# hkust-vgd/nerfstyle

Hardware: AMD Instinct MI355X
Metric: train Mrays/sec (higher is better)
Workload: dtype f16

## Files before the change

nerfstyle_amd/csrc/field_bwd_gout.hip:

```cpp
#include "field_bwd.h"

template <int CD>
__device__ __forceinline__ void field_wgrad_mfma4(f4v &c0, f4v &c1, f4v &c2, f4v &c3, s4v a0, s4v b0, s4v a1, s4v b1, s4v a2,
                                                  s4v b2, s4v a3, s4v b3) {
    if (CD == NSR_F16)
        asm volatile("s_nop 1\n\t"
                     "v_mfma_f32_16x16x16_f16 %0, %4, %5, %0\n\t"
                     "v_mfma_f32_16x16x16_f16 %1, %6, %7, %1\n\t"
                     "v_mfma_f32_16x16x16_f16 %2, %8, %9, %2\n\t"
                     "v_mfma_f32_16x16x16_f16 %3, %10, %11, %3"
                     : "+a"(c0), "+a"(c1), "+a"(c2), "+a"(c3)
                     : "v"(a0), "v"(b0), "v"(a1), "v"(b1), "v"(a2), "v"(b2), "v"(a3), "v"(b3));
    else
        asm volatile("s_nop 1\n\t"
                     "v_mfma_f32_16x16x16_bf16 %0, %4, %5, %0\n\t"
                     "v_mfma_f32_16x16x16_bf16 %1, %6, %7, %1\n\t"
                     "v_mfma_f32_16x16x16_bf16 %2, %8, %9, %2\n\t"
                     "v_mfma_f32_16x16x16_bf16 %3, %10, %11, %3"
                     : "+a"(c0), "+a"(c1), "+a"(c2), "+a"(c3)
                     : "v"(a0), "v"(b0), "v"(a1), "v"(b1), "v"(a2), "v"(b2), "v"(a3), "v"(b3));
}
template <int NT>
__device__ __forceinline__ void field_wgrad_settle(f4v (&acc)[NT]) {
    static_assert(NT % 4 == 0, "accumulators come in blocks of four");
#pragma unroll
    for (int k = 0; k < NT; k += 4)
        asm volatile("s_nop 15\n\ts_nop 3" : "+a"(acc[k]), "+a"(acc[k + 1]), "+a"(acc[k + 2]), "+a"(acc[k + 3]));
}
template <int CD, int NG, int NA>
__device__ __forceinline__ void field_wgrad(f4v (&acc)[NG * NA], const s4v (&Gt)[NG], const s4v (&At)[NA]) {
    static_assert((NG * NA) % 4 == 0, "accumulators come in blocks of four");
#pragma unroll
    for (int j = 0; j < NG * NA; j += 4)
        field_wgrad_mfma4<CD>(acc[j], acc[j + 1], acc[j + 2], acc[j + 3], Gt[j / NA], At[j % NA], Gt[(j + 1) / NA],
                              At[(j + 1) % NA], Gt[(j + 2) / NA], At[(j + 2) % NA], Gt[(j + 3) / NA], At[(j + 3) % NA]);
}

constexpr int TR_DEPTH = 4;
template <int CD>
__device__ __forceinline__ void field_tr4p(const s8v (&x)[2], s4v ident, s4v (&out)[4]) {
    const s4v in[4] = {mm_lo(x[0]), mm_hi(x[0]), mm_lo(x[1]), mm_hi(x[1])};
    mm_transpose16_n<CD, 4, TR_DEPTH>(in, ident, out);
}
template <int CD>
__device__ __forceinline__ void field_tr5p(const s8v (&x)[2], s4v y, s4v ident, s4v (&out)[4], s4v (&yt)[1]) {
    const s4v in[5] = {mm_lo(x[0]), mm_hi(x[0]), mm_lo(x[1]), mm_hi(x[1]), y};
    s4v o[5];
    mm_transpose16_n<CD, 5, TR_DEPTH>(in, ident, o);
    out[0] = o[0]; out[1] = o[1]; out[2] = o[2]; out[3] = o[3]; yt[0] = o[4];
}
template <int CD>
__device__ __forceinline__ void field_tr6p(const s8v (&x)[2], s4v y, s4v z, s4v ident, s4v (&out)[4], s4v (&yt)[1], s4v (&zt)[1]) {
    const s4v in[6] = {mm_lo(x[0]), mm_hi(x[0]), mm_lo(x[1]), mm_hi(x[1]), y, z};
    s4v o[6];
    mm_transpose16_n<CD, 6, TR_DEPTH>(in, ident, o);
    out[0] = o[0]; out[1] = o[1]; out[2] = o[2]; out[3] = o[3]; yt[0] = o[4]; zt[0] = o[5];
}

template <typename TT, int CD, bool FEATS, bool DIRS = false>
__global__ void __launch_bounds__(BWD_THREADS)
k_field_bwd_gout(FieldBwdArgsOf<DIRS> b) {
    constexpr int FWT = FW_IMAGE<DIRS>;
    const float *const dirs = field_dirs_of(b);
    extern __shared__ __attribute__((aligned(16))) char smem[];
    short *wl = reinterpret_cast<short *>(smem);
    short *wt = wl + FWT;
    NsrLevel *lds_lv = reinterpret_cast<NsrLevel *>(smem + (size_t)(FWT + BW_TOTAL) * 2);
    const FieldArgs &a = b.f;
    field_build_fw<CD, false, DIRS>(wl, a.params);
    field_build_bw<CD>(wt, a.params);
    if (threadIdx.x < 16) lds_lv[threadIdx.x] = a.lv[threadIdx.x];
    __syncthreads();

    const uint32_t Mc = FIELD_COUNT(a);
    const uint32_t ntiles = (Mc + 15) / 16;
    const int lane = threadIdx.x & 63, wave = __builtin_amdgcn_readfirstlane((int)(threadIdx.x >> 6));
    const int s = lane & 15, g = lane >> 4;
    const TT *tables = reinterpret_cast<const TT *>(a.tables);
    const uint32_t lb = field_logical_block();
    const uint32_t tpb = (ntiles + gridDim.x - 1) / gridDim.x;
    const uint32_t t_begin = lb * tpb;
    const uint32_t t_end = min(t_begin + tpb, ntiles);
    const s4v ident = mm_identity_frag<CD>(lane);
    const int nc = (int)b.nc;
    const bool td = b.train_density != 0, tc = b.train_color != 0;
    f4v w_r3[4], w_r2[16], w_r1[4], w_c1b[4], w_c1a[8], w_k2[4], w_k1[8], w_d2[4], w_d1[8];
    f4v w_sh[4];
    {
        const f4v z = {0.f, 0.f, 0.f, 0.f};
        if constexpr (DIRS) { w_sh[0] = z; w_sh[1] = z; w_sh[2] = z; w_sh[3] = z; }
#pragma unroll
        for (int q4 = 0; q4 < 4; q4++) { w_r3[q4] = z; w_r1[q4] = z; w_c1b[q4] = z; w_k2[q4] = z; w_d2[q4] = z; }
#pragma unroll
        for (int q8 = 0; q8 < 8; q8++) { w_c1a[q8] = z; w_k1[q8] = z; w_d1[q8] = z; }
#pragma unroll
        for (int q16 = 0; q16 < 16; q16++) w_r2[q16] = z;
    }

    struct TileIn {
        float x0, x1, x2;
        s8v xd, xc;
        float gsig;
        float grgb[4];
    };
    auto fetch_idx = [&](uint32_t tile) -> uint32_t {
        const uint32_t m = tile * 16 + s;
        if (a.perm) return a.perm[min(m, Mc - 1u)];
        return m < Mc ? m : 0u;
    };
    auto load_tile = [&](uint32_t tile, uint32_t buf_idx) {
        TileIn r;
        const size_t mc = buf_idx;
        r.x0 = a.xyzs[mc * 3 + 0];
        r.x1 = a.xyzs[mc * 3 + 1];
        r.x2 = a.xyzs[mc * 3 + 2];
        r.gsig = b.grad_sigmas[mc];
        const float *gp = b.grad_rgbs + mc * a.C_ch;
        if (a.C_ch == 8) {
            const float4 t4 = reinterpret_cast<const float4 *>(gp)[g & 1];
            r.grgb[0] = t4.x; r.grgb[1] = t4.y; r.grgb[2] = t4.z; r.grgb[3] = t4.w;
        } else {
#pragma unroll
            for (int e = 0; e < 4; e++) r.grgb[e] = gp[(uint32_t)(4 * g + e) < a.C_ch ? 4 * g + e : 0];
        }
        if (FEATS) {
            const s8v *fi = reinterpret_cast<const s8v *>(a.feats) + ((size_t)tile * 64 + lane) * 2;
            r.xd = fi[0];
            r.xc = fi[1];
        }
        return r;
    };
    const uint32_t wchunk = (t_end > t_begin ? (t_end - t_begin + BWD_THREADS / 64 - 1) / (BWD_THREADS / 64) : 0u);
    const uint32_t w_begin = min(t_begin + wave * wchunk, t_end), w_end = min(w_begin + wchunk, t_end);
    TileIn cur;
    uint32_t idx_cur = 0, idx_next = 0;
    if (w_begin < w_end) {
        idx_cur = fetch_idx(w_begin);
        cur = load_tile(w_begin, idx_cur);
        idx_next = w_begin + 1 < w_end ? fetch_idx(w_begin + 1) : idx_cur;
    }
    float4 gout_v[4];
    uint32_t gout_m = 0;
    bool gout_valid = false;
    auto gout_store = [&]() {
        if (gout_valid) {
#pragma unroll
            for (int i = 0; i < 4; i++) {
                const int lv_i = (i < 2 ? 2 * g : 8 + 2 * g) + (i & 1);
                b.gout[(size_t)gout_m * 16 + lv_i] = gout_v[i];
            }
        }
        gout_valid = false;
    };
    bool ch_on[4], ch_rgb[4], ch_cls[4];
#pragma unroll
    for (int e = 0; e < 4; e++) {
        const int ch = 4 * g + e;
        ch_on[e] = a.C_ch == 8 ? g < 2 : (uint32_t)ch < a.C_ch;
        ch_rgb[e] = (uint32_t)ch < a.C_ch && ch < 3;
        ch_cls[e] = (uint32_t)ch < a.C_ch && ch >= 3;
    }
    s8v wq[4];
    s4v wq16[4];
    mm_queue32<4>(wq, wl + FW_D1, lane);
    for (uint32_t tile = w_begin; tile < w_end; tile++) {
        const uint32_t m = tile * 16 + s;
        const bool valid = m < Mc;
        asm volatile("" ::: "memory");
        asm volatile("" :: "v"(cur.x0), "v"(cur.x1), "v"(cur.x2), "v"(cur.gsig), "v"(cur.grgb[0]), "v"(cur.grgb[1]),
                     "v"(cur.grgb[2]), "v"(cur.grgb[3]), "v"(cur.xd), "v"(cur.xc), "v"(idx_next));
        float dv[3] = {0.f, 0.f, 0.f};
        if constexpr (DIRS) { dv[0] = dirs[(size_t)idx_cur * 3 + 0]; dv[1] = dirs[(size_t)idx_cur * 3 + 1]; dv[2] = dirs[(size_t)idx_cur * 3 + 2]; }
        const float u0 = field_unit(cur.x0, a.bmin[0], a.bsize[0]);
        const float u1 = field_unit(cur.x1, a.bmin[1], a.bsize[1]);
        const float u2 = field_unit(cur.x2, a.bmin[2], a.bsize[2]);
        const bool live = valid && (u0 >= 0 && u0 <= 1 && u1 >= 0 && u1 <= 1 && u2 >= 0 && u2 <= 1);
        const float cur_gsig = valid ? cur.gsig : 0.f;
        float cur_grgb[4];
#pragma unroll
        for (int e = 0; e < 4; e++) cur_grgb[e] = (valid && ch_on[e]) ? cur.grgb[e] : 0.f;
        if (!FEATS) field_encode<TT, CD, false>(lds_lv, tables, u0, u1, u2, live, g, cur.xd, cur.xc, a.fast_levels);

        f4v gxd[2], gxc[2];
        s8v xd[1] = {cur.xd}, xc[1] = {cur.xc};
        f4v h[4];
        s8v hd[2], hk[2], hc[2], hr1[2], hr2[2];
        f4v logit[1], c1[1], rgb[1];
        mm_layer32_q<CD, 4, 1>(wq, wl + FW_D1, lane, xd, h);
        mm_queue32<2>(wq, wl + FW_D2, lane);
        gout_store();
        const TileIn nxt = load_tile(min(tile + 1, w_end - 1), idx_next);
        const uint32_t idx_nn = fetch_idx(min(tile + 2, w_end - 1));
        mm_pack64<CD, true, true>(h, hd);
        mm_layer32_q<CD, 1, 2>(wq, wl + FW_D2, lane, hd, logit);
        mm_queue32<4>(wq, wl + FW_K1, lane);
        mm_layer32_q<CD, 4, 1>(wq, wl + FW_K1, lane, xc, h);
        mm_queue32<4>(wq, wl + FW_C1A, lane);
        mm_pack64<CD, true, true>(h, hk);
        mm_layer32_q<CD, 4, 1>(wq, wl + FW_C1A, lane, xc, h);
        mm_queue32<2>(wq, wl + FW_C1B, lane);
        mm_pack64<CD, true, true>(h, hc);
        mm_layer32_q<CD, 1, 2>(wq, wl + FW_C1B, lane, hc, c1);
        s4v shb = {};
        if constexpr (DIRS) mm_queue32<4>(wq, wl + FW_R1, lane);
        else mm_queue16<4>(wq16, wl + FW_R1, lane);
        const s4v c1b = mm_round4<CD, false>(c1[0]);
        if constexpr (DIRS) {
            shb = mm_round4<CD, false>(field_sh4(g, dv[0], dv[1], dv[2]));
            const s8v b1[1] = {mm_cat(c1b, shb)};
            mm_layer32_q<CD, 4, 1>(wq, wl + FW_R1, lane, b1, h);
        } else {
            mm_layer16_q<CD, 4>(wq16, c1b, h);
        }
        mm_queue32<8>(wq, wl + FW_R2, lane);
        mm_pack64<CD, true, true>(h, hr1);
        mm_layer32_q<CD, 4, 2>(wq, wl + FW_R2, lane, hr1, h);
        mm_queue32<2>(wq, wl + FW_R3, lane);
        mm_pack64<CD, true, true>(h, hr2);
        mm_layer32_q<CD, 1, 2>(wq, wl + FW_R3, lane, hr2, rgb);
        mm_queue16<4>(wq16, wt + BW_R3T, lane);

        s4v dyd, dyr, dyk;
        {
            float gd[4] = {0.f, 0.f, 0.f, 0.f}, gr[4] = {0.f, 0.f, 0.f, 0.f}, gk[4] = {0.f, 0.f, 0.f, 0.f};
            {
                const float x = logit[0][0];
                const float d = cur_gsig * a.density_scale * expf(fminf(fmaxf(x, -15.0f), 15.0f));
                gd[0] = (valid && g == 0) ? d : 0.f;
            }
#pragma unroll
            for (int e = 0; e < 4; e++) {
                const float gv = cur_grgb[e];
                if (e < 3) {
                    const float sg = field_sigmoid(rgb[0][e]);
                    const float d = gv * sg * (1.0f - sg);
                    gr[e] = (valid && ch_rgb[e]) ? d : 0.f;
                }
                gk[e] = (valid && ch_cls[e]) ? gv : 0.f;
            }
#pragma unroll
            for (int e = 0; e < 4; e++) { dyd[e] = MM<CD>::cvt(gd[e]); dyr[e] = MM<CD>::cvt(gr[e]); dyk[e] = MM<CD>::cvt(gk[e]); }
        }

        s8v g2[2], g1[2];
        s4v gc1;
        {
            mm_layer16_q<CD, 4>(wq16, dyr, h);
            mm_queue32<8>(wq, wt + BW_R2T, lane);
            field_mask_pack<CD, true>(h, hr2, g2);
            mm_layer32_q<CD, 4, 2>(wq, wt + BW_R2T, lane, g2, h);
            mm_queue32<2>(wq, wt + BW_R1T, lane);
            field_mask_pack<CD, true>(h, hr1, g1);
            f4v t1[1];
            mm_layer32_q<CD, 1, 2>(wq, wt + BW_R1T, lane, g1, t1);
            mm_queue16<4>(wq16, wt + BW_C1BT, lane);
            gc1 = mm_round4<CD, false>(t1[0]);
            s4v hr2t[4], hr1t[4], g2t[4], g1t[4], dyrt[1], c1t[1];
            field_tr5p<CD>(hr2, dyr, ident, hr2t, dyrt);
            field_wgrad<CD>(w_r3, dyrt, hr2t);
            field_tr4p<CD>(g2, ident, g2t);
            field_tr4p<CD>(hr1, ident, hr1t);
            field_wgrad<CD>(w_r2, g2t, hr1t);
            if constexpr (DIRS) {
                s4v sht[1];
                field_tr6p<CD>(g1, c1b, shb, ident, g1t, c1t, sht);
                field_wgrad<CD>(w_r1, g1t, c1t);
                field_wgrad<CD>(w_sh, g1t, sht);
            } else {
                field_tr5p<CD>(g1, c1b, ident, g1t, c1t);
                field_wgrad<CD>(w_r1, g1t, c1t);
            }
        }
        s4v xct[2], xdt[2];
        {
            const s8v xcd[2] = {xc[0], xd[0]};
            s4v xt[4];
            field_tr4p<CD>(xcd, ident, xt);
            xct[0] = xt[0]; xct[1] = xt[1]; xdt[0] = xt[2]; xdt[1] = xt[3];
        }

        {
            s8v gh[2];
            s4v ght[4], hct[4], gc1t[1];
            mm_layer16_q<CD, 4>(wq16, gc1, h);
            mm_queue32<4>(wq, wt + BW_C1AT, lane);
            field_mask_pack<CD, true>(h, hc, gh);
            mm_layer32_q<CD, 2, 2>(wq, wt + BW_C1AT, lane, gh, gxc);
            mm_queue16<4>(wq16, wt + BW_K2T, lane);
            field_tr5p<CD>(hc, gc1, ident, hct, gc1t);
            field_wgrad<CD>(w_c1b, gc1t, hct);
            field_tr4p<CD>(gh, ident, ght);
            field_wgrad<CD>(w_c1a, ght, xct);
        }
        {
            s8v gh[2];
            s4v ght[4], hkt[4], dykt[1];
            mm_layer16_q<CD, 4>(wq16, dyk, h);
            mm_queue32<4>(wq, wt + BW_K1T, lane);
            field_mask_pack<CD, true>(h, hk, gh);
            mm_layer32_q<CD, 2, 2, true>(wq, wt + BW_K1T, lane, gh, gxc);
            mm_queue16<4>(wq16, wt + BW_D2T, lane);
            field_tr5p<CD>(hk, dyk, ident, hkt, dykt);
            field_wgrad<CD>(w_k2, dykt, hkt);
            field_tr4p<CD>(gh, ident, ght);
            field_wgrad<CD>(w_k1, ght, xct);
        }
        {
            s8v gh[2];
            s4v ght[4], hdt[4], dydt[1];
            mm_layer16_q<CD, 4>(wq16, dyd, h);
            mm_queue32<4>(wq, wt + BW_D1T, lane);
            field_mask_pack<CD, true>(h, hd, gh);
            mm_layer32_q<CD, 2, 2>(wq, wt + BW_D1T, lane, gh, gxd);
            mm_queue32<4>(wq, wl + FW_D1, lane);
            field_tr5p<CD>(hd, dyd, ident, hdt, dydt);
            field_wgrad<CD>(w_d2, dydt, hdt);
            field_tr4p<CD>(gh, ident, ght);
            field_wgrad<CD>(w_d1, ght, xdt);
        }

        if (td || tc) {
            float4 sg[4];
#pragma unroll
            for (int i = 0; i < 4; i++) {
                const int t = i >> 1, e0 = 2 * (i & 1);
                sg[i] = live ? make_float4(gxd[t][e0], gxd[t][e0 + 1], gxc[t][e0], gxc[t][e0 + 1]) : make_float4(0.f, 0.f, 0.f, 0.f);
            }
#pragma unroll
            for (int i = 0; i < 4; i++) gout_v[i] = sg[i];
            gout_m = idx_cur;
            gout_valid = valid;
        }
        cur = nxt;
        idx_cur = idx_next; idx_next = idx_nn;
    }
    gout_store();
        field_wgrad_settle(w_r3); field_wgrad_settle(w_r2); field_wgrad_settle(w_r1); field_wgrad_settle(w_c1b);
        field_wgrad_settle(w_c1a); field_wgrad_settle(w_k2); field_wgrad_settle(w_k1); field_wgrad_settle(w_d2);
        field_wgrad_settle(w_d1);
        if constexpr (DIRS) field_wgrad_settle(w_sh);

    if (b.grad_mlp) {
        f4v *const red = reinterpret_cast<f4v *>(smem);
#define NSR_RED_ALL(OP)                                                                                              \
        OP(w_r3, 0, 4) OP(w_r2, 4, 16) OP(w_r1, 20, 4) OP(w_c1b, 24, 4) OP(w_c1a, 28, 8) OP(w_k2, 36, 4) OP(w_k1, 40, 8)     \
        OP(w_d2, 48, 4) OP(w_d1, 52, 8)
        __syncthreads();
        for (int w = 0; w < BWD_THREADS / 64; w++) {
            if (wave == w) {
                if (w == 0) {
#define NSR_RED_ST(arr, base, n) _Pragma("unroll") for (int i = 0; i < n; i++) red[((base) + i) * 64 + lane] = arr[i];
                    NSR_RED_ALL(NSR_RED_ST)
                    if constexpr (DIRS) { NSR_RED_ST(w_sh, 60, 4) }
#undef NSR_RED_ST
                } else {
#define NSR_RED_ADD(arr, base, n) _Pragma("unroll") for (int i = 0; i < n; i++) red[((base) + i) * 64 + lane] += arr[i];
                    NSR_RED_ALL(NSR_RED_ADD)
                    if constexpr (DIRS) { NSR_RED_ADD(w_sh, 60, 4) }
#undef NSR_RED_ADD
                }
            }
            __syncthreads();
        }
        if (wave == 0) {
#define NSR_RED_LD(arr, base, n) _Pragma("unroll") for (int i = 0; i < n; i++) arr[i] = red[((base) + i) * 64 + lane];
            NSR_RED_ALL(NSR_RED_LD)
            if constexpr (DIRS) { NSR_RED_LD(w_sh, 60, 4) }
#undef NSR_RED_LD
            float *gm = b.grad_mlp;
            if constexpr (DIRS) field_wgrad_flush<4, 1>(gm + P_SH, 16, 0, 64, w_sh, lane);
            field_wgrad_flush<1, 4>(gm + P_R3, 64, 0, 3, w_r3, lane);
            field_wgrad_flush<4, 4>(gm + P_R2, 64, 0, 64, w_r2, lane);
            field_wgrad_flush<4, 1>(gm + P_R1, 16, 0, 64, w_r1, lane);
            field_wgrad_flush<1, 4>(gm + P_C1B, 64, 0, 16, w_c1b, lane);
            field_wgrad_flush<4, 2>(gm + P_C1A, 32, 0, 64, w_c1a, lane);
            field_wgrad_flush<1, 4>(gm + P_K2, 64, CLASS_ROW_SHIFT, nc, w_k2, lane);
            field_wgrad_flush<4, 2>(gm + P_K1, 32, 0, 64, w_k1, lane);
            field_wgrad_flush<1, 4>(gm + P_D2, 64, 0, 1, w_d2, lane);
            field_wgrad_flush<4, 2>(gm + P_D1, 32, 0, 64, w_d1, lane);
        }
#undef NSR_RED_ALL
    }
}

constexpr int COLOR_THREADS = 512;
template <int CD, bool DIRS = false>
__global__ void __launch_bounds__(COLOR_THREADS)
k_field_bwd_color(FieldBwdArgsOf<DIRS> b) {
    constexpr int AHEAD = 4;
    const float *const dirs = field_dirs_of(b);
    extern __shared__ __attribute__((aligned(16))) char smem[];
    short *wl = reinterpret_cast<short *>(smem);
    short *wt = wl + FW_IMAGE<DIRS>;
    const FieldArgs &a = b.f;
    field_build_fw<CD, false, DIRS>(wl, a.params);
    field_build_bw<CD>(wt, a.params);
    __syncthreads();
    const uint32_t Mc = FIELD_COUNT(a);
    const uint32_t ntiles = (Mc + 15) / 16;
    const int lane = threadIdx.x & 63, wave = threadIdx.x >> 6;
    const int s = lane & 15, g = lane >> 4;
    const uint32_t lb = field_logical_block();
    const uint32_t tpb = (ntiles + gridDim.x - 1) / gridDim.x;
    const uint32_t t_begin = lb * tpb;
    const uint32_t t_end = min(t_begin + tpb, ntiles);
    for (uint32_t tile = t_begin + wave; tile < t_end; tile += COLOR_THREADS / 64) {
        const uint32_t mpos = tile * 16 + s;
        const bool valid = mpos < Mc;
        const uint32_t m = a.perm[min(mpos, Mc - 1u)];
        const float u0 = field_unit(a.xyzs[(size_t)m * 3 + 0], a.bmin[0], a.bsize[0]);
        const float u1 = field_unit(a.xyzs[(size_t)m * 3 + 1], a.bmin[1], a.bsize[1]);
        const float u2 = field_unit(a.xyzs[(size_t)m * 3 + 2], a.bmin[2], a.bsize[2]);
        const bool live = valid && field_in_unit_cube(u0, u1, u2);
        float grgb[4];
        {
            const float *gp = b.grad_rgbs + (size_t)m * a.C_ch;
            if (a.C_ch == 8) {
                const float4 t4 = reinterpret_cast<const float4 *>(gp)[g & 1];
                grgb[0] = t4.x; grgb[1] = t4.y; grgb[2] = t4.z; grgb[3] = t4.w;
            } else {
#pragma unroll
                for (int e = 0; e < 4; e++) grgb[e] = gp[(uint32_t)(4 * g + e) < a.C_ch ? 4 * g + e : 0];
            }
#pragma unroll
            for (int e = 0; e < 4; e++)
                if (!(valid && (a.C_ch == 8 ? g < 2 : (uint32_t)(4 * g + e) < a.C_ch))) grgb[e] = 0.f;
        }
        const s8v xc[1] = {(reinterpret_cast<const s8v *>(a.feats) + ((size_t)tile * 64 + lane) * 2)[1]};
        f4v h[4];
        s8v hk[2], hc[2], hr1[2], hr2[2];
        f4v c1[1], rgb[1];
        mm_layer32<CD, 4, 1, AHEAD>(wl + FW_K1, lane, xc, h);
        mm_pack64<CD, true, true>(h, hk);
        mm_layer32<CD, 4, 1, AHEAD>(wl + FW_C1A, lane, xc, h);
        mm_pack64<CD, true, true>(h, hc);
        mm_layer32<CD, 1, 2, AHEAD>(wl + FW_C1B, lane, hc, c1);
        const s4v c1b = mm_round4<CD, false>(c1[0]);
        if constexpr (DIRS) {
            const s8v b1[1] = {mm_cat(c1b, field_sh_frag<CD>(dirs, m, valid, g))};
            mm_layer32<CD, 4, 1, AHEAD>(wl + FW_R1, lane, b1, h);
        } else {
            mm_layer16<CD, 4, AHEAD>(wl + FW_R1, lane, c1b, h);
        }
        mm_pack64<CD, true, true>(h, hr1);
        mm_layer32<CD, 4, 2, AHEAD>(wl + FW_R2, lane, hr1, h);
        mm_pack64<CD, true, true>(h, hr2);
        mm_layer32<CD, 1, 2, AHEAD>(wl + FW_R3, lane, hr2, rgb);
        s4v dyr, dyk;
#pragma unroll
        for (int e = 0; e < 4; e++) {
            const int ch = 4 * g + e;
            float gr = 0.f, gk = 0.f;
            if (valid && (uint32_t)ch < a.C_ch) {
                if (ch < 3) {
                    const float sg = field_sigmoid(rgb[0][e]);
                    gr = grgb[e] * sg * (1.0f - sg);
                } else {
                    gk = grgb[e];
                }
            }
            dyr[e] = MM<CD>::cvt(gr);
            dyk[e] = MM<CD>::cvt(gk);
        }
        s8v g2[2], g1[2], gh[2];
        f4v t1[1], gxc[2];
        mm_layer16<CD, 4, AHEAD>(wt + BW_R3T, lane, dyr, h);
        field_mask_pack<CD, true>(h, hr2, g2);
        mm_layer32<CD, 4, 2, AHEAD>(wt + BW_R2T, lane, g2, h);
        field_mask_pack<CD, true>(h, hr1, g1);
        mm_layer32<CD, 1, 2, AHEAD>(wt + BW_R1T, lane, g1, t1);
        const s4v gc1 = mm_round4<CD, false>(t1[0]);
        mm_layer16<CD, 4, AHEAD>(wt + BW_C1BT, lane, gc1, h);
        field_mask_pack<CD, true>(h, hc, gh);
        mm_layer32<CD, 2, 2, AHEAD>(wt + BW_C1AT, lane, gh, gxc);
        mm_layer16<CD, 4, AHEAD>(wt + BW_K2T, lane, dyk, h);
        field_mask_pack<CD, true>(h, hk, gh);
        mm_layer32_acc<CD, 2, 2, AHEAD>(wt + BW_K1T, lane, gh, gxc);
        if (valid) {
#pragma unroll
            for (int i = 0; i < 4; i++) {
                const int t = i >> 1, e0 = 2 * (i & 1);
                const int lv_i = (i < 2 ? 2 * g : 8 + 2 * g) + (i & 1);
                b.gout[(size_t)m * 16 + lv_i] = live ? make_float4(0.f, 0.f, gxc[t][e0], gxc[t][e0 + 1]) : make_float4(0.f, 0.f, 0.f, 0.f);
            }
        }
    }
}
template <int CD>
static int field_bwd_launch_color(const FieldBwdArgs &b, hipStream_t s, const float *dirs) {
    const size_t lds = (size_t)(FW_IMAGE<false> + BW_TOTAL) * 2, lds_dirs = (size_t)(FW_IMAGE<true> + BW_TOTAL) * 2;
    const uint32_t ntiles = (b.f.M + 15) / 16;
    uint32_t nb = (ntiles + 63) / 64;
    if (nb > 512) nb = 512;
    if (nb == 0) nb = 1;
    if (dirs) {
        const FieldBwdDirsArgs bd = field_bwd_with_dirs(b, dirs);
        return nsr_launch_lds<k_field_bwd_color<CD, true>>(lds_dirs, dim3(nb), dim3(COLOR_THREADS), lds_dirs, s, bd);
    }
    return nsr_launch_lds<k_field_bwd_color<CD>>(lds, dim3(nb), dim3(COLOR_THREADS), lds, s, b);
}

int nsr_field_bwd_launch_gout(const FieldBwdArgs &b, int table_dtype, int compute_dtype, bool feats, dim3 grid, hipStream_t s,
                              const float *dirs) {
    if (b.grad_mlp == nullptr && !b.train_density && b.train_color && feats && b.f.perm != nullptr) {
        if (compute_dtype == NSR_F16) return field_bwd_launch_color<NSR_F16>(b, s, dirs);
        if (compute_dtype == NSR_BF16) return field_bwd_launch_color<NSR_BF16>(b, s, dirs);
    }
    return field_bwd_dispatch(table_dtype, compute_dtype, feats, [&](auto tt, auto cd, auto ft) {
        if (dirs) {
            const FieldBwdDirsArgs bd = field_bwd_with_dirs(b, dirs);
            return nsr_launch_lds<k_field_bwd_gout<decltype(tt), cd(), ft(), true>>(BWD_LDS_BYTES_DIRS, grid, dim3(BWD_THREADS),
                                                                                    BWD_LDS_BYTES_DIRS, s, bd);
        }
        return nsr_launch_lds<k_field_bwd_gout<decltype(tt), cd(), ft()>>(BWD_LDS_BYTES, grid, dim3(BWD_THREADS), BWD_LDS_BYTES, s, b);
    });
}
```

Measured before the change: 23.98.

## Interleave mask-pack VALU steps into weight-gradient MFMA chains and reorder layers

```diff
diff --git a/nerfstyle_amd/csrc/field_bwd_gout.hip b/nerfstyle_amd/csrc/field_bwd_gout.hip
--- a/nerfstyle_amd/csrc/field_bwd_gout.hip
+++ b/nerfstyle_amd/csrc/field_bwd_gout.hip
@@ -35,6 +35,74 @@
         field_wgrad_mfma4<CD>(acc[j], acc[j + 1], acc[j + 2], acc[j + 3], Gt[j / NA], At[j % NA], Gt[(j + 1) / NA],
                               At[(j + 1) % NA], Gt[(j + 2) / NA], At[(j + 2) % NA], Gt[(j + 3) / NA], At[(j + 3) % NA]);
 }
+
+template <int CD>
+__device__ __forceinline__ void field_wgrad_mfma_head(f4v &c0, s4v a0, s4v b0, s4v a1, s4v b1, s4v a2, s4v b2, s4v a3, s4v b3) {
+    if (CD == NSR_F16)
+        asm volatile("s_nop 1\n\tv_mfma_f32_16x16x16_f16 %0, %1, %2, %0"
+                     : "+a"(c0) : "v"(a0), "v"(b0), "v"(a1), "v"(b1), "v"(a2), "v"(b2), "v"(a3), "v"(b3));
+    else
+        asm volatile("s_nop 1\n\tv_mfma_f32_16x16x16_bf16 %0, %1, %2, %0"
+                     : "+a"(c0) : "v"(a0), "v"(b0), "v"(a1), "v"(b1), "v"(a2), "v"(b2), "v"(a3), "v"(b3));
+}
+template <int CD>
+__device__ __forceinline__ void field_wgrad_mfma_next(f4v &c, s4v a, s4v b) {
+    if (CD == NSR_F16) asm volatile("v_mfma_f32_16x16x16_f16 %0, %1, %2, %0" : "+a"(c) : "v"(a), "v"(b));
+    else asm volatile("v_mfma_f32_16x16x16_bf16 %0, %1, %2, %0" : "+a"(c) : "v"(a), "v"(b));
+}
+template <int CD>
+struct FieldMaskPackSteps {
+    static constexpr int PIECES = 16;
+    const f4v (&gacc)[4];
+    const s8v (&act)[2];
+    uint32_t gp[8], m[8], o[8];
+    __device__ __forceinline__ FieldMaskPackSteps(const f4v (&g)[4], const s8v (&a)[2]) : gacc(g), act(a) {}
+    __device__ __forceinline__ uint32_t act_word(int w) const { return __builtin_bit_cast(uint4, act[w >> 2])[w & 3]; }
+    __device__ __forceinline__ uint32_t cvt_pair(int w) const {
+        const f4v &g = gacc[w >> 1];
+        const int e = 2 * (w & 1);
+        if (CD == NSR_F16) {
+            typedef _Float16 hh2 __attribute__((ext_vector_type(2)));
+            const hh2 hp = {(_Float16)g[e], (_Float16)g[e + 1]};
+            return __builtin_bit_cast(uint32_t, hp);
+        } else {
+            typedef __bf16 bb2 __attribute__((ext_vector_type(2)));
+            const bb2 bp = {(__bf16)g[e], (__bf16)g[e + 1]};
+            return __builtin_bit_cast(uint32_t, bp);
+        }
+    }
+    __device__ __forceinline__ void step(int i) {
+        const int w = 4 * (i >> 3) + 2 * (i & 1), k = (i >> 1) & 3;
+        if (k == 0)
+            asm("v_pk_sub_i16 %0, 0, %2 clamp\n\tv_pk_sub_i16 %1, 0, %3 clamp"
+                : "=&v"(m[w]), "=&v"(m[w + 1]) : "v"(act_word(w)), "v"(act_word(w + 1)));
+        else if (k == 1)
+            asm("v_pk_ashrrev_i16 %0, 15, %0 op_sel_hi:[0,1]\n\tv_pk_ashrrev_i16 %1, 15, %1 op_sel_hi:[0,1]" : "+v"(m[w]), "+v"(m[w + 1]));
+        else if (k == 2) { gp[w] = cvt_pair(w); gp[w + 1] = cvt_pair(w + 1); }
+        else { o[w] = gp[w] & m[w]; o[w + 1] = gp[w + 1] & m[w + 1]; }
+    }
+    __device__ __forceinline__ void result(s8v (&out)[2]) const {
+        out[0] = __builtin_bit_cast(s8v, make_uint4(o[0], o[1], o[2], o[3]));
+        out[1] = __builtin_bit_cast(s8v, make_uint4(o[4], o[5], o[6], o[7]));
+    }
+};
+template <int CD, int NG, int NA, int P0, int PN, typename H>
+__device__ __forceinline__ void field_wgrad_hosting(f4v (&acc)[NG * NA], const s4v (&Gt)[NG], const s4v (&At)[NA], H &host) {
+    constexpr int N = NG * NA;
+    static_assert(N % 4 == 0, "accumulators come in blocks of four");
+#pragma unroll
+    for (int j = 0; j < N; j++) {
+        if (j % 4 == 0)
+            field_wgrad_mfma_head<CD>(acc[j], Gt[j / NA], At[j % NA], Gt[(j + 1) / NA], At[(j + 1) % NA], Gt[(j + 2) / NA],
+                                      At[(j + 2) % NA], Gt[(j + 3) / NA], At[(j + 3) % NA]);
+        else
+            field_wgrad_mfma_next<CD>(acc[j], Gt[j / NA], At[j % NA]);
+#pragma unroll
+        for (int p = P0 + j * PN / N; p < P0 + (j + 1) * PN / N; p++) host.step(p);
+        __builtin_amdgcn_sched_barrier(0);
+    }
+}
+
 
 constexpr int TR_DEPTH = 4;
 template <int CD>
@@ -242,34 +310,37 @@
             for (int e = 0; e < 4; e++) { dyd[e] = MM<CD>::cvt(gd[e]); dyr[e] = MM<CD>::cvt(gr[e]); dyk[e] = MM<CD>::cvt(gk[e]); }
         }
 
+        using MaskPack = FieldMaskPackSteps<CD>;
         s8v g2[2], g1[2];
         s4v gc1;
+        s4v g1t[4], c1t[1], sht[1];
         {
+            s4v hr2t[4], hr1t[4], g2t[4], dyrt[1];
             mm_layer16_q<CD, 4>(wq16, dyr, h);
             mm_queue32<8>(wq, wt + BW_R2T, lane);
-            field_mask_pack<CD, true>(h, hr2, g2);
+            field_tr5p<CD>(hr2, dyr, ident, hr2t, dyrt);
+            {
+                MaskPack mp(h, hr2);
+                __builtin_amdgcn_sched_barrier(0);
+                field_wgrad_hosting<CD, 1, 4, 0, 16>(w_r3, dyrt, hr2t, mp);
+                mp.result(g2);
+            }
             mm_layer32_q<CD, 4, 2>(wq, wt + BW_R2T, lane, g2, h);
             mm_queue32<2>(wq, wt + BW_R1T, lane);
-            field_mask_pack<CD, true>(h, hr1, g1);
+            field_tr4p<CD>(g2, ident, g2t);
+            field_tr4p<CD>(hr1, ident, hr1t);
+            {
+                MaskPack mp(h, hr1);
+                __builtin_amdgcn_sched_barrier(0);
+                field_wgrad_hosting<CD, 4, 4, 0, 16>(w_r2, g2t, hr1t, mp);
+                mp.result(g1);
+            }
             f4v t1[1];
             mm_layer32_q<CD, 1, 2>(wq, wt + BW_R1T, lane, g1, t1);
             mm_queue16<4>(wq16, wt + BW_C1BT, lane);
             gc1 = mm_round4<CD, false>(t1[0]);
-            s4v hr2t[4], hr1t[4], g2t[4], g1t[4], dyrt[1], c1t[1];
-            field_tr5p<CD>(hr2, dyr, ident, hr2t, dyrt);
-            field_wgrad<CD>(w_r3, dyrt, hr2t);
-            field_tr4p<CD>(g2, ident, g2t);
-            field_tr4p<CD>(hr1, ident, hr1t);
-            field_wgrad<CD>(w_r2, g2t, hr1t);
-            if constexpr (DIRS) {
-                s4v sht[1];
-                field_tr6p<CD>(g1, c1b, shb, ident, g1t, c1t, sht);
-                field_wgrad<CD>(w_r1, g1t, c1t);
-                field_wgrad<CD>(w_sh, g1t, sht);
-            } else {
-                field_tr5p<CD>(g1, c1b, ident, g1t, c1t);
-                field_wgrad<CD>(w_r1, g1t, c1t);
-            }
+            if constexpr (DIRS) field_tr6p<CD>(g1, c1b, shb, ident, g1t, c1t, sht);
+            else field_tr5p<CD>(g1, c1b, ident, g1t, c1t);
         }
         s4v xct[2], xdt[2];
         {
@@ -279,42 +350,62 @@
             xct[0] = xt[0]; xct[1] = xt[1]; xdt[0] = xt[2]; xdt[1] = xt[3];
         }
 
+        s4v ght[4];
         {
             s8v gh[2];
-            s4v ght[4], hct[4], gc1t[1];
+            s4v hct[4], gc1t[1];
             mm_layer16_q<CD, 4>(wq16, gc1, h);
             mm_queue32<4>(wq, wt + BW_C1AT, lane);
-            field_mask_pack<CD, true>(h, hc, gh);
+            field_tr5p<CD>(hc, gc1, ident, hct, gc1t);
+            {
+                MaskPack mp(h, hc);
+                __builtin_amdgcn_sched_barrier(0);
+                if constexpr (DIRS) {
+                    field_wgrad_hosting<CD, 4, 1, 0, 5>(w_r1, g1t, c1t, mp);
+                    field_wgrad_hosting<CD, 4, 1, 5, 5>(w_sh, g1t, sht, mp);
+                    field_wgrad_hosting<CD, 1, 4, 10, 6>(w_c1b, gc1t, hct, mp);
+                } else {
+                    field_wgrad_hosting<CD, 4, 1, 0, 8>(w_r1, g1t, c1t, mp);
+                    field_wgrad_hosting<CD, 1, 4, 8, 8>(w_c1b, gc1t, hct, mp);
+                }
+                mp.result(gh);
+            }
             mm_layer32_q<CD, 2, 2>(wq, wt + BW_C1AT, lane, gh, gxc);
             mm_queue16<4>(wq16, wt + BW_K2T, lane);
-            field_tr5p<CD>(hc, gc1, ident, hct, gc1t);
-            field_wgrad<CD>(w_c1b, gc1t, hct);
             field_tr4p<CD>(gh, ident, ght);
-            field_wgrad<CD>(w_c1a, ght, xct);
         }
         {
             s8v gh[2];
-            s4v ght[4], hkt[4], dykt[1];
+            s4v hkt[4], dykt[1];
             mm_layer16_q<CD, 4>(wq16, dyk, h);
             mm_queue32<4>(wq, wt + BW_K1T, lane);
-            field_mask_pack<CD, true>(h, hk, gh);
+            field_tr5p<CD>(hk, dyk, ident, hkt, dykt);
+            {
+                MaskPack mp(h, hk);
+                __builtin_amdgcn_sched_barrier(0);
+                field_wgrad_hosting<CD, 4, 2, 0, 10>(w_c1a, ght, xct, mp);
+                field_wgrad_hosting<CD, 1, 4, 10, 6>(w_k2, dykt, hkt, mp);
+                mp.result(gh);
+            }
             mm_layer32_q<CD, 2, 2, true>(wq, wt + BW_K1T, lane, gh, gxc);
             mm_queue16<4>(wq16, wt + BW_D2T, lane);
-            field_tr5p<CD>(hk, dyk, ident, hkt, dykt);
-            field_wgrad<CD>(w_k2, dykt, hkt);
             field_tr4p<CD>(gh, ident, ght);
-            field_wgrad<CD>(w_k1, ght, xct);
         }
         {
             s8v gh[2];
-            s4v ght[4], hdt[4], dydt[1];
+            s4v hdt[4], dydt[1];
             mm_layer16_q<CD, 4>(wq16, dyd, h);
             mm_queue32<4>(wq, wt + BW_D1T, lane);
-            field_mask_pack<CD, true>(h, hd, gh);
+            field_tr5p<CD>(hd, dyd, ident, hdt, dydt);
+            {
+                MaskPack mp(h, hd);
+                __builtin_amdgcn_sched_barrier(0);
+                field_wgrad_hosting<CD, 4, 2, 0, 10>(w_k1, ght, xct, mp);
+                field_wgrad_hosting<CD, 1, 4, 10, 6>(w_d2, dydt, hdt, mp);
+                mp.result(gh);
+            }
             mm_layer32_q<CD, 2, 2>(wq, wt + BW_D1T, lane, gh, gxd);
             mm_queue32<4>(wq, wl + FW_D1, lane);
-            field_tr5p<CD>(hd, dyd, ident, hdt, dydt);
-            field_wgrad<CD>(w_d2, dydt, hdt);
             field_tr4p<CD>(gh, ident, ght);
             field_wgrad<CD>(w_d1, ght, xdt);
         }
```

After: 24.12, median of 6. About the same (+0.6%).
